# alex-petrenko/megaverse

Measured on AMD Instinct MI355X. Metric: agent observations/sec (whole node), TowerBuilding 128x128 obs, random policy, higher is better.
Workload: dtype f32

## Files before the change

### megaverse_amd/csrc/mv_raster.hip

```cpp
#include <hip/hip_runtime.h>
#include <hip/hip_ext.h>
#include <math.h>
#include <stdlib.h>

#include <algorithm>
#include <cstring>
#include <numeric>
#include <type_traits>
#include <vector>
#include <stdio.h>

#include "../../include/megaverse_hip.h"
#include "mv_frame.h"
#include "mv_math.h"
#include "mv_raster.h"
#include "mv_rearrange.h"
#include "mv_types.h"
#include "mv_union.h"

namespace mv {

namespace {

template <bool ANYZERO>
// ... 504 lines not shown
            const int py = pyBase + TILE_H * k;
            if constexpr (CHW) put_px(frame_out<true>(obs, frame, W, H, false), px, py, rgba);
            else if (px < W && py < H) out[(size_t)py * W + px] = rgba;
        }
    }
}

namespace {

#ifndef MV_GLIST_WAVES_NP2
#define MV_GLIST_WAVES_NP2 5
#endif
#ifndef MV_GLIST_WAVES_NP1
#define MV_GLIST_WAVES_NP1 6
#endif
constexpr int GLIST_WAVES_NP2 = MV_GLIST_WAVES_NP2, GLIST_WAVES_NP1 = MV_GLIST_WAVES_NP1;
#ifndef MV_FAST_PPL_DEFAULT
#define MV_FAST_PPL_DEFAULT 2
#endif
constexpr float SPEC_COS2 = 0.97f * 0.97f;

#ifndef MV_PIXEL_PLAIN
#define PIXEL_STORE(dst, v) __builtin_nontemporal_store((uint32_t)(v), &(dst))
#else
#define PIXEL_STORE(dst, v) ((dst) = (v))
#endif

struct FastArgs {
    const unsigned char *vis_hdr;
    const Prim *vis_prims;
    const short4 *vis_rects;
    const int *hist, *list;
    int num_agents, vis_stride, frames;
    const float *stage_rewards, *stage_true;
    const uint8_t *stage_done;
    float *pub_rewards, *pub_true;
    uint8_t *pub_done;
    int pub_n;
#ifdef MV_RASTER_TIMING
    unsigned long long *rdbg;
#endif
    int *hist_done;
    int wg_total;
    int tail_div, tail_split;
    int planar;
};

__device__ __forceinline__ void fast_publish(const FastArgs &fa, int blk)
{
    if (fa.pub_n == 0) return;
    const int i = blk * (int)blockDim.x + (int)threadIdx.x;
    if (i >= fa.pub_n) return;
    fa.pub_rewards[i] = fa.stage_rewards[i];
    const int e = i / fa.num_agents;
    if (fa.stage_done[e]) fa.pub_true[i] = fa.stage_true[i];
    if (i < fa.pub_n / fa.num_agents) fa.pub_done[i] = fa.stage_done[i];
}

__device__ __forceinline__ unsigned long long uniform_u64(unsigned long long v)
{
    const unsigned lo = (unsigned)__builtin_amdgcn_readfirstlane((unsigned)v), hi = (unsigned)__builtin_amdgcn_readfirstlane((unsigned)(v >> 32));
    return ((unsigned long long)hi << 32) | lo;
}

__device__ __forceinline__ float uniform_f32(float v)
{
// ... 155 lines not shown
    unsigned rgba = 0xff000000u;
    if (best <= (KEY_FAR | POS_MASK)) {
        const int pos = (int)(best & POS_MASK);
        rgba = shade_rec<SHAPES>(s_vis[2 * pos], s_vis[2 * pos + 1], __uint_as_float((best & ~POS_MASK) + KEY_NEAR),
                                 bn, s_hdr, camv, viewer, dw, inv, dcx, dcy, a2, ldc);
    }
    return rgba;
}

struct FastFrame { int frame, part, viewer, nVis, split; };

__host__ __device__ inline int tail_frames(int frames, int div) { return (frames / div) & ~7; }

template <int MAXVIS, bool GLIST = false, int NT = 256>
__device__ __forceinline__ FastFrame fast_prologue(const FastArgs &fa, int blk, int W, int H, int split,
                                                   float4 *s_vis, short4 *s_rect, float *s_hdr, float4 *s_col,
                                                   float4 *s_row, float2 *s_rowq, float *s_colq, unsigned char *s_cls = nullptr)
{
    const int A = fa.num_agents;
    const int tid = threadIdx.x, lane = tid & 63, wave = __builtin_amdgcn_readfirstlane(tid >> 6);
    int position, part;
    {
        int b = blk, first = 0, frames = fa.frames;
        if (fa.tail_div) {
            const int q = tail_frames(frames, fa.tail_div), head = frames - q;
            if (b < split * head) frames = head;
            else { b -= split * head; first = head; split = fa.tail_split; frames = q; }
        }
        const int per = 8 * split, group = b / per, r = b - group * per;
        position = group * 8 + (r & 7); part = r >> 3;
        if (group * 8 + 8 > frames) { const int nf = frames - group * 8; position = group * 8 + r % nf; part = r / nf; }
        position += first;
    }
    __shared__ int s_wsum[4], s_frame, s_lastWG;
    {
        static_assert(LPT_SUBS == 4, "the bin's counters are read as one int4");
        const bool binThread = NT == 256 || tid < LPT_BUCKETS;
        const int4 c0 = binThread ? *reinterpret_cast<const int4 *>(fa.hist + (LPT_BUCKETS - 1 - tid) * LPT_SUBS) : make_int4(0, 0, 0, 0);
        const int h = (c0.x + c0.y) + (c0.z + c0.w);
        int x = h;
#pragma unroll
        for (int off = 1; off < 64; off <<= 1) {
            const int y = __shfl_up(x, off, 64);
            if (lane >= off) x += y;
        }
        if (lane == 63 && binThread) s_wsum[wave] = x;
        __syncthreads();
        int base = 0;
        for (int w = 0; w < wave && w < 4; ++w) base += s_wsum[w];
        const int end = base + x, start = end - h;
        if (binThread && position >= start && position < end) {
            const int cs[LPT_SUBS] = {c0.x, c0.y, c0.z, c0.w};
            int off = position - start, sub = 0;
#pragma unroll
            for (int q = 0; q < LPT_SUBS - 1; ++q)
                if (sub == q && off >= cs[q]) { off -= cs[q]; sub = q + 1; }
            s_frame = fa.list[(size_t)((LPT_BUCKETS - 1 - tid) * LPT_SUBS + sub) * lpt_sub_capacity(fa.frames) + off];
        }
        __syncthreads();
    }
#ifdef MV_HIST_FENCE
    if (tid == 0) s_lastWG = fa.hist_done != nullptr && __hip_atomic_fetch_add(fa.hist_done, 1, __ATOMIC_ACQ_REL, __HIP_MEMORY_SCOPE_AGENT) == fa.wg_total - 1;
#else
    if (tid == 0) s_lastWG = fa.hist_done != nullptr && __hip_atomic_fetch_add(fa.hist_done, 1, __ATOMIC_RELAXED, __HIP_MEMORY_SCOPE_AGENT) == fa.wg_total - 1;
#endif
    const int frame = __builtin_amdgcn_readfirstlane(s_frame);
    const int viewer = frame % A;
    const float *gh = reinterpret_cast<const float *>(fa.vis_hdr + (size_t)frame * FRAME_HDR_BYTES);
    const int nVis = __builtin_amdgcn_readfirstlane(min(__float_as_int(gh[FH_COUNT]), (int)MAXVIS));

    if (tid < FH_FLOATS) s_hdr[tid] = gh[tid];
    {
        const float4 *src = reinterpret_cast<const float4 *>(fa.vis_prims + (size_t)frame * fa.vis_stride);
        if (!GLIST) for (int i = tid; i < nVis * 2; i += NT) s_vis[i] = src[i];
        else
            for (int i = tid; i < nVis; i += NT) {
                const unsigned ml = __float_as_uint(reinterpret_cast<const float *>(src)[8 * i + 3]);
                const unsigned fl = (ml >> 4) & 15u;
                s_cls[i] = (ml & 15u) != (unsigned)PRIM_BOX ? 4 : fl == 0u ? 0 : fl > (unsigned)MAX_AGENTS ? (unsigned char)(fl - (unsigned)MAX_AGENTS) : 4;
            }
        const short4 *rs = fa.vis_rects + (size_t)frame * fa.vis_stride;
        for (int i = tid; i < nVis; i += NT) s_rect[i] = rs[i];
        const float *c = gh + FH_CAM + FH_CAM_STRIDE * viewer + 3;
        for (int i = tid; i < W; i += NT) {
            const float dcx = (((float(i) + 0.5f) / float(W)) * 2.0f - 1.0f) * TAN_HALF_FOV;
            s_col[i] = make_float4(dcx, c[0] * dcx, c[3] * dcx, c[6] * dcx);
            s_colq[i] = dcx * dcx;
        }
        for (int j = tid; j < H; j += NT) {
            const float dcy = (((float(j) + 0.5f) / float(H)) * 2.0f - 1.0f) * TAN_HALF_FOV_Y;
            s_row[j] = make_float4(dcy, c[1] * dcy, c[4] * dcy, c[7] * dcy);
            s_rowq[j] = make_float2(dcy * dcy + 1.0f, 4.0f * dcy - 2.0f);
        }
// ... 17 lines not shown
    const float tf = __builtin_fminf(__builtin_fminf(fx * inv.x, fy * inv.y), fz * inv.z);
    const unsigned key = ((__float_as_uint(tn) - KEY_NEAR) & depthMask) | (unsigned)pos;
    return tn <= tf ? key : ~0u;
}

template <unsigned POS_MASK, int NP, int SGN = -1>
__device__ __forceinline__ void box_run(unsigned long long m, int k, const V3 (&inv)[NP], const float4 *s_vis, unsigned (&best)[NP])
{
    if (!m) return;
    int p0 = __ffsll((long long)m) - 1 + 64 * k, p1 = 0;
    m &= m - 1;
    float4 lo0 = s_vis[2 * p0], hi0 = s_vis[2 * p0 + 1], lo1 = lo0, hi1 = hi0;
    unsigned depthMask = ~POS_MASK;
    asm volatile("" : "+v"(depthMask));
    for (;;) {
        bool more = m != 0ull;
        if (more) { p1 = __ffsll((long long)m) - 1 + 64 * k; m &= m - 1; lo1 = s_vis[2 * p1]; hi1 = s_vis[2 * p1 + 1]; }
#pragma unroll
        for (int j = 0; j < NP; ++j) best[j] = min(best[j], SGN >= 0 ? box_key_signed<POS_MASK, (SGN >= 0 ? SGN : 0)>(inv[j], lo0, hi0, p0, depthMask)
             : box_key<POS_MASK>(inv[j], lo0, hi0, p0, depthMask));
        if (!more) break;
        more = m != 0ull;
        if (more) { p0 = __ffsll((long long)m) - 1 + 64 * k; m &= m - 1; lo0 = s_vis[2 * p0]; hi0 = s_vis[2 * p0 + 1]; }
#pragma unroll
        for (int j = 0; j < NP; ++j) best[j] = min(best[j], SGN >= 0 ? box_key_signed<POS_MASK, (SGN >= 0 ? SGN : 0)>(inv[j], lo1, hi1, p1, depthMask)
             : box_key<POS_MASK>(inv[j], lo1, hi1, p1, depthMask));
        if (!more) break;
    }
}

}

constexpr float PLANAR_MARGIN = 2e-4f;
enum : unsigned { TC_EMPTY = 0, TC_PLANAR = 1, TC_PLANAR_SPEC = 2, TC_OVERLAY = 3, TC_GENERAL = 4 };
constexpr int CLS_MAX_TILES = 128;

template <int TH, int NT>
__device__ __forceinline__ void classify_tiles(uint4 *s_tile, float4 *s_line, const float4 *s_vis, const short4 *s_rect,
                                               const float *s_hdr, const float *camv, int nVis, unsigned long long wb0,
                                               int W, int H, int part, int split, int tilesX, int numTiles,
                                                       int perWG, bool overlayOn, int *s_cnt, unsigned *s_txy, bool bulkClear)
{
    constexpr int NW = NT / 64;
    constexpr int PPR = 16 / NW;
    const int tid = threadIdx.x, lane = tid & 63, wave = __builtin_amdgcn_readfirstlane(tid >> 6);
    if (tid < CLS_MAX_TILES) s_tile[tid] = make_uint4(0u, 0u, 0u, 0u);
    if (tid < 8) s_cnt[tid] = 0;
    const float sx = 2.0f * TAN_HALF_FOV / float(W), ox = (1.0f / float(W) - 1.0f) * TAN_HALF_FOV;
    const float sy = 2.0f * TAN_HALF_FOV_Y / float(H), oy = (1.0f / float(H) - 1.0f) * TAN_HALF_FOV_Y;
    const int q = lane & 15, es = lane >> 4;
    const int ek = min(q >> 2, 2);
    int em = ek + 1 + ((q >> 1) & 1);
    em = em >= 3 ? em - 3 : em;
    const bool ehi = q & 1, eactive = q < 12;
    const float Ak = camv[3 + 3 * ek] * sx, Bk = camv[4 + 3 * ek] * sy, Ck = (camv[3 + 3 * ek] * ox + camv[4 + 3 * ek] * oy) - camv[5 + 3 * ek];
    const float Am = camv[3 + 3 * em] * sx, Bm = camv[4 + 3 * em] * sy, Cm = (camv[3 + 3 * em] * ox + camv[4 + 3 * em] * oy) - camv[5 + 3 * em];
    float4 *myLines = s_line + 16 * PPR * wave;
    constexpr float WX = float(TILE_W - 1), WY = float(TH - 1);
    __syncthreads();
    constexpr int CH = CLS_MAX_TILES / 64;
    int tX0[CH], tY0[CH], tX1[CH], tY1[CH];
    bool tvalid[CH];
    unsigned mlo[CH], mhi[CH], cover[CH];
#pragma unroll
    for (int c = 0; c < CH; ++c) {
        const int u = 64 * c + lane;
        const int tile = ((u >> 2) * split + part) * 4 + (u & 3);
        tvalid[c] = u < perWG && tile < numTiles;
        const int tyi = tile / tilesX, txi = tile - tyi * tilesX;
        tX0[c] = txi * TILE_W; tY0[c] = tyi * TH;
        tX1[c] = min(tX0[c] + TILE_W, W) - 1; tY1[c] = min(tY0[c] + TH, H) - 1;
        mlo[c] = mhi[c] = cover[c] = 0u;
    }
    for (int base = PPR * wave; base < nVis; base += 16) {
        const int P = min(base + min(es, PPR - 1), nVis - 1);
        const bool isBox = es < PPR && base + es < nVis && ((wb0 >> P) & 1ull) != 0ull;
        const float4 lo4 = s_vis[2 * P], hi4 = s_vis[2 * P + 1];
        const float lok = ek == 0 ? lo4.x : ek == 1 ? lo4.y : lo4.z, hik = ek == 0 ? hi4.x : ek == 1 ? hi4.y : hi4.z;
        const float lom = em == 0 ? lo4.x : em == 1 ? lo4.y : lo4.z, him = em == 0 ? hi4.x : em == 1 ? hi4.y : hi4.z;
        const float bnd = ehi ? him : lom;
        const bool cand = isBox && eactive && (lok > 0.0f || hik < 0.0f);
        const float pk = lok > 0.0f ? lok : hik;
        const float far1 = (__builtin_fmaxf(__builtin_fabsf(lo4.x), __builtin_fabsf(hi4.x)) + __builtin_fmaxf(__builtin_fabsf(lo4.y), __builtin_fabsf(hi4.y))) +
                           __builtin_fmaxf(__builtin_fabsf(lo4.z), __builtin_fabsf(hi4.z));
        const bool coverOK = cand && __builtin_fabsf(pk) >= 4.0f * NEAR_Z && far1 <= 0.5f * FAR_Z;
        const float sg = ((pk > 0.0f) != ehi) ? 1.0f : -1.0f;
        const float ea = sg * (pk * Am - bnd * Ak), eb = sg * (pk * Bm - bnd * Bk), ec = sg * (pk * Cm - bnd * Ck);
        const float mg = PLANAR_MARGIN * (__builtin_fabsf(pk) + __builtin_fabsf(bnd));
        const float cin = ((ec + __builtin_fminf(0.0f, ea * WX)) + __builtin_fminf(0.0f, eb * WY)) - mg;
        const float span = (__builtin_fabsf(ea) * WX + __builtin_fabsf(eb) * WY) + 2.0f * mg;
        if (es < PPR) myLines[lane] = cand ? make_float4(ea, eb, cin, span) : make_float4(0.0f, 0.0f, -1.0f, 0.0f);
        const unsigned long long candMask = __ballot(cand), coverMask = __ballot(coverOK);
        __builtin_amdgcn_fence(__ATOMIC_RELEASE, "wavefront");
        __builtin_amdgcn_wave_barrier();
        __builtin_amdgcn_fence(__ATOMIC_ACQUIRE, "wavefront");
#pragma unroll
        for (int sl = 0; sl < PPR; ++sl) {
            const int Q = base + sl;
            if (Q >= nVis) break;
            const uint2 rr = *reinterpret_cast<const uint2 *>(&s_rect[Q]);
            const bool worldBox = (wb0 >> Q) & 1ull;
#pragma unroll
            for (int c = 0; c < CH; ++c) {
                if (64 * c >= perWG) break;
                const bool ov = tvalid[c] & ((int)(rr.x & 0xffffu) <= tX1[c]) & ((int)(rr.x >> 16) >= tX0[c])
                                             & ((int)(rr.y & 0xffffu) <= tY1[c]) & ((int)(rr.y >> 16) >= tY0[c]);
                if (!__any(ov)) continue;
                bool hit = ov;
                unsigned cov = 0u;
                if (worldBox) {
                    const float fx0 = float(tX0[c]), fy0 = float(tY0[c]);
                    bool missAll = true;
#pragma unroll
                    for (int f = 0; f < 3; ++f) {
                        if (!((candMask >> (16 * sl + 4 * f)) & 1ull)) continue;
                        bool ins = true, mis = false;
#pragma unroll
                        for (int e = 0; e < 4; ++e) {
                            const float4 L = myLines[16 * sl + 4 * f + e];
                            const float g = __builtin_fmaf(L.x, fx0, __builtin_fmaf(L.y, fy0, L.z));
                            ins = ins && g >= 0.0f;
                            mis = mis || g + L.w <= 0.0f;
                        }
                        if (ins && ((coverMask >> (16 * sl + 4 * f)) & 1ull)) cov = (unsigned)f + 1u;
                        missAll = missAll && mis;
                    }
                    hit = ov && !missAll;
                }
                if (hit) {
                    if (Q < 32) mlo[c] |= 1u << Q; else mhi[c] |= 1u << (Q - 32);
                    cover[c] |= cov;
                }
            }
        }
        __builtin_amdgcn_fence(__ATOMIC_RELEASE, "wavefront");
        __builtin_amdgcn_wave_barrier();
        __builtin_amdgcn_fence(__ATOMIC_ACQUIRE, "wavefront");
    }
#pragma unroll
    for (int c = 0; c < CH; ++c)
        if (tvalid[c]) {
            const int u = 64 * c + lane;
            if (mlo[c]) atomicOr(&s_tile[u].x, mlo[c]);
            if (mhi[c]) atomicOr(&s_tile[u].y, mhi[c]);
            if (cover[c]) atomicOr(&s_tile[u].z, cover[c]);
        }
    __syncthreads();
    {
        const float hx = 0.5f * WX * sx, hy = 0.5f * WY * sy;
        const float r2 = hx * hx + hy * hy;
        const float cosT = 0.965f * __builtin_amdgcn_sqrtf(__builtin_fmaxf(1.0f - r2, 0.0f)) - 0.2623f * __builtin_amdgcn_sqrtf(r2);
        const bool usable = r2 < 0.5f && cosT > 0.0f;
        const float cosT2 = cosT * cosT;
        const float L0 = s_hdr[FH_LREL + 0], L1 = s_hdr[FH_LREL + 1], L2 = s_hdr[FH_LREL + 2];
        const unsigned long long nonBox = __ballot(lane < nVis && (__float_as_uint(s_vis[2 * min(lane, max(nVis - 1, 0))].w) & 15u) != (unsigned)PRIM_BOX);
#pragma unroll
        for (int c = 0; c < CH; ++c) {
            if (wave != (c % NW) || !tvalid[c]) continue;
            const int u = 64 * c + lane;
            const uint4 tc = s_tile[u];
            const unsigned long long m = ((unsigned long long)tc.y << 32) | tc.x, wbm = m & wb0, others = m & ~wb0;
            unsigned info = TC_GENERAL;
            if (m == 0ull) info = TC_EMPTY;
            else if (wbm != 0ull && (wbm & (wbm - 1ull)) == 0ull && tc.z != 0u) {
                const int pos = __ffsll((long long)wbm) - 1, k = (int)tc.z - 1;
                if (others == 0ull) {
                    bool maybe = true;
                    if (usable) {
                        const float lok = reinterpret_cast<const float *>(s_vis)[8 * pos + k], hik = reinterpret_cast<const float *>(s_vis)[8 * pos + 4 + k];
                        const float plane = lok > 0.0f ? lok : hik;
                        const float m0 = k == 0 ? 2.0f * plane - L0 : L0, m1 = k == 1 ? 2.0f * plane - L1 : L1, m2 = k == 2 ? 2.0f * plane - L2 : L2;
                        const float xc = float(tX0[c]) + 0.5f * WX, yc = float(tY0[c]) + 0.5f * WY;
                        const float dcx = sx * xc + ox, dcy = sy * yc + oy;
                        const float d0 = (camv[3] * dcx + camv[4] * dcy) - camv[5], d1 = (camv[6] * dcx + camv[7] * dcy) - camv[8],
// ... 5 lines not shown
                    info = (maybe ? (unsigned)TC_PLANAR_SPEC : (unsigned)TC_PLANAR) | ((unsigned)k << 3) | ((unsigned)pos << 5);
                } else if ((others & nonBox) == 0ull && overlayOn) info = (unsigned)TC_OVERLAY | ((unsigned)k << 3) | ((unsigned)pos << 5);
            }
            if (info == TC_GENERAL) {
                const float xa = float(tX0[c]), xb = float(tX1[c]), ya = float(tY0[c]), yb = float(tY1[c]);
                unsigned sg = 8u;
#pragma unroll
                for (int a = 0; a < 3; ++a) {
                    const float Aa = camv[3 + 3 * a] * sx, Ba = camv[4 + 3 * a] * sy, Ca = (camv[3 + 3 * a] * ox + camv[4 + 3 * a] * oy) - camv[5 + 3 * a];
                    const float v00 = __builtin_fmaf(Aa, xa, __builtin_fmaf(Ba, ya, Ca)), v10 = __builtin_fmaf(Aa, xb, __builtin_fmaf(Ba, ya, Ca));
                    const float v01 = __builtin_fmaf(Aa, xa, __builtin_fmaf(Ba, yb, Ca)), v11 = __builtin_fmaf(Aa, xb, __builtin_fmaf(Ba, yb, Ca));
                    const float lo4 = __builtin_fminf(__builtin_fminf(v00, v10), __builtin_fminf(v01, v11)),
                                                      hi4 = __builtin_fmaxf(__builtin_fmaxf(v00, v10), __builtin_fmaxf(v01, v11));
                    if (hi4 < -1e-4f) sg |= 1u << a;
                    else if (!(lo4 > 1e-4f)) sg = 0u;
                    if (sg == 0u) break;
                }
                info |= sg << 11;
            }
            s_tile[u].w = info;
            const unsigned tclass = info & 7u, cat = tclass == TC_GENERAL ? 0u : tclass == TC_OVERLAY ? 1u
                    : tclass == TC_PLANAR_SPEC ? 2u : tclass == TC_PLANAR ? 3u : 4u;
            const bool runs = tclass == TC_PLANAR || tclass == TC_PLANAR_SPEC || (tclass == TC_EMPTY && !bulkClear);
            const unsigned txy = (unsigned)tX0[c] | ((unsigned)tY0[c] << 16);
            const unsigned prevInfo = (unsigned)__shfl_up((int)info, 1, 64), prevTxy = (unsigned)__shfl_up((int)txy, 1, 64);
            const bool natHead = !runs || lane == 0 || prevInfo != info || prevTxy + (unsigned)TILE_W != txy;
            const unsigned long long nat = __ballot(natHead), below = nat & ((2ull << lane) - 1ull);
            const int posInRun = lane - (63 - __clzll((long long)below));
            const bool head = natHead || (posInRun & 7) == 0;
            const unsigned long long heads = __ballot(head), valid = __ballot(true), above = lane < 63 ? heads >> (lane + 1) : 0ull;
            const int nextHead = above ? lane + __ffsll((long long)above) : 64;
            const int len = min(nextHead, (int)__popcll(valid)) - lane;
            s_tile[u].z = head ? cat | ((unsigned)len << 3) | ((unsigned)atomicAdd(&s_cnt[cat], 1) << 7) : 7u;
            s_txy[u] = txy;
        }
        __syncthreads();
    }
}

template <int NP, bool SPEC, class PO>
__device__ __forceinline__ void planar_run(int pos, int k, int n, const float4 *s_vis, const float *s_hdr, const float4 *s_col, const float4 *s_row,
                                           const float2 *s_rowq, const float *s_colq, float nzk, int tx0, int ty0, int lane, const PO &po)
{
    const int W = po.W, H = po.H;
    const float lok = uniform_f32(reinterpret_cast<const float *>(s_vis)[8 * pos + k]),
                                  hik = uniform_f32(reinterpret_cast<const float *>(s_vis)[8 * pos + 4 + k]);
    const float plane = lok > 0.0f ? lok : hik;
    const unsigned color = (unsigned)__builtin_amdgcn_readfirstlane(__float_as_uint(reinterpret_cast<const float *>(s_vis)[8 * pos + 7]));
    const float cr = float((color >> 16) & 255u), cg = float((color >> 8) & 255u), cb = float(color & 255u);
    const float lk = uniform_f32(s_hdr[FH_LREL + k]);
    const float lks = plane > 0.0f ? lk : 0.0f - lk;
    int lpx = lane;
    asm volatile("" : "+v"(lpx));
    const int lx = lpx & (TILE_W - 1), py0 = ty0 + lpx / TILE_W;
    float rowk[NP];
    float2 rq[NP];
#pragma unroll
    for (int j = 0; j < NP; ++j) {
        const int pyc = min(py0 + TILE_H * j, H - 1);
        rowk[j] = reinterpret_cast<const float *>(s_row)[4 * pyc + 1 + k];
        rq[j] = s_rowq[pyc];
    }
#pragma unroll 1
    for (int q = 0; q < n; ++q) {
        const int px = tx0 + TILE_W * q + lx, pxc = min(px, W - 1);
        const float colk = reinterpret_cast<const float *>(s_col)[4 * pxc + 1 + k];
        const float cq = s_colq[pxc];
// ... 148 lines not shown
    const unsigned long long wbm = mv0 & wb0;
    switch (signs) {
    case 8: box_run<POS_MASK, NP, 0>(wbm, 0, inv, s_vis, best); break;
    case 9: box_run<POS_MASK, NP, 1>(wbm, 0, inv, s_vis, best); break;
    case 10: box_run<POS_MASK, NP, 2>(wbm, 0, inv, s_vis, best); break;
    case 11: box_run<POS_MASK, NP, 3>(wbm, 0, inv, s_vis, best); break;
    case 12: box_run<POS_MASK, NP, 4>(wbm, 0, inv, s_vis, best); break;
    case 13: box_run<POS_MASK, NP, 5>(wbm, 0, inv, s_vis, best); break;
    case 14: box_run<POS_MASK, NP, 6>(wbm, 0, inv, s_vis, best); break;
    case 15: box_run<POS_MASK, NP, 7>(wbm, 0, inv, s_vis, best); break;
    default: box_run<POS_MASK, NP>(wbm, 0, inv, s_vis, best); break;
    }
    unsigned long long rest = mv0 & ~wb0;
    while (rest) {
        const int pos = __ffsll((long long)rest) - 1;
        rest &= rest - 1;
#pragma unroll
        for (int j = 0; j < NP; ++j) {
            V3 n = v3(0, 0, 0);
            const unsigned key = fast_other<SHAPES, POS_MASK>(pos, s_vis, s_hdr, camv, viewer, dw[j], dcx, dcy[j], n);
            if (key < best[j]) { best[j] = key; bn[j] = n; }
        }
    }
#pragma unroll
    for (int j = 0; j < NP; ++j) {
        const unsigned rgba = fast_shade<SHAPES, POS_MASK>(best[j], bn[j], s_vis, s_hdr, camv, viewer, dw[j], inv[j], dcx, dcy[j], a2[j], ldc[j]);
        put_px(po, px, py0 + TILE_H * j, rgba);
    }
}

constexpr int fast_lds_bytes(int maxvis) { return 40 * maxvis + 4 * FH_FLOATS; }
constexpr int glist_lds_bytes(int maxvis) { return 9 * maxvis + 4 * FH_FLOATS; }

#ifdef MV_RASTER_TIMING
#define RT_COUNT(i, n) do { const unsigned long long n_ = (unsigned long long)(n); if (fa.rdbg && lane == 0) atomicAdd(fa.rdbg + (size_t)16384 * 4 * 8 + (i), n_); } while (0)
#else
#define RT_COUNT(i, n) do { } while (0)
#endif
template <bool SHAPES, unsigned POS_MASK, int NP, bool LISTED, class PO>
__device__ __forceinline__ void classified_tile(const FastArgs &fa, const int u, const int tx0, const int ty0, const uint4 *s_tile,
                                                const float4 *s_vis, const float *s_hdr, const float *camv, int viewer,
                                            const float4 *s_col, const float4 *s_row, const float2 *s_rowq,
                                                    const float *s_colq, float nzm0, float nzm1, float nzm2, unsigned long long wb0,
                                            int lane, const PO &po)
{
    const unsigned info = (unsigned)__builtin_amdgcn_readfirstlane(s_tile[u].w), tclass = info & 7u;
    const int run = LISTED ? (int)(((unsigned)__builtin_amdgcn_readfirstlane(s_tile[u].z) >> 3) & 15u) : 1;
    RT_COUNT(0, run);
    if (tclass == TC_EMPTY) {
        RT_COUNT(1, run);
        for (int q = 0; q < run; ++q) clear_tile<NP>(po, tx0 + TILE_W * q, ty0, lane);
        return;
    }
    if (LISTED && tclass <= TC_PLANAR_SPEC) {
        const int k = (int)((info >> 3) & 3u), posA = (int)(info >> 5);
        const float nzk = k == 0 ? nzm0 : k == 1 ? nzm1 : nzm2;
        RT_COUNT(2, run);
        RT_COUNT(12, tclass == TC_PLANAR ? run : 0);
        if (tclass == TC_PLANAR) planar_run<NP, false>(posA, k, run, s_vis, s_hdr, s_col, s_row, s_rowq, s_colq, nzk, tx0, ty0, lane, po);
        else planar_run<NP, true>(posA, k, run, s_vis, s_hdr, s_col, s_row, s_rowq, s_colq, nzk, tx0, ty0, lane, po);
        return;
    }
    int lpx = lane;
    asm volatile("" : "+v"(lpx));
    const int px = tx0 + (lpx & (TILE_W - 1)), py0 = ty0 + lpx / TILE_W;
    if (tclass <= TC_OVERLAY) {
#if defined(MV_RASTER_DEBUG_SKIP) && MV_RASTER_DEBUG_SKIP == 3
        return;
#endif
        const int k = (int)((info >> 3) & 3u), posA = (int)(info >> 5);
        const float nzk = k == 0 ? nzm0 : k == 1 ? nzm1 : nzm2;
// ... 43 lines not shown
    unsigned long long rt_[6];
    rt_[0] = __builtin_amdgcn_s_memtime(); rt_[5] = __builtin_amdgcn_s_memrealtime();
#define RT_MARK(i) rt_[i] = __builtin_amdgcn_s_memtime()
#else
#define RT_MARK(i) do { } while (0)
#endif
    fast_publish(fa, blk);
    const FastFrame ff = fast_prologue<MAXVIS, false, NT>(fa, blk, W, H, split, s_vis, s_rect, s_hdr, s_col, s_row, s_rowq, s_colq);
    RT_MARK(1);
    const int frame = ff.frame, part = ff.part, viewer = ff.viewer, nVis = ff.nVis;
    split = ff.split;

    const float *camv = s_hdr + FH_CAM + FH_CAM_STRIDE * viewer;
    const float nzm0 = uniform_f32(-camv[3 + 2]), nzm1 = uniform_f32(-camv[3 + 5]), nzm2 = uniform_f32(-camv[3 + 8]);
    uint32_t *out = obs + (size_t)frame * W * H;
    const int tilesX = (W + TILE_W - 1) / TILE_W, tilesY = (H + TH - 1) / TH;
    const int numTiles = tilesX * tilesY;
    PixOutT<CHW> po;
    if constexpr (CHW) po = frame_out<true>(obs, frame, W, H, (W % TILE_W) == 0 && (H % TH) == 0);
    else {
        po.rsrc = __builtin_amdgcn_make_buffer_rsrc(out,  0, W * H * 4, 0x00020000);
        po.W = W; po.H = H; po.W4 = 4 * W;
        po.edgeless = (W % TILE_W) == 0 && (H % TH) == 0;
    }

    uint2 rr0 = make_uint2(0u, 0u);
    if (NP == 1) rr0 = *reinterpret_cast<const uint2 *>(&s_rect[min(lane, max(nVis - 1, 0))]);
    const unsigned long long wb0 = uniform_u64(*reinterpret_cast<const unsigned long long *>(s_hdr + FH_WB));

    constexpr bool PLANAR = !HEXF && CLS;
    static_assert(!PLANAR || (MAXVIS == 256 && CLS_MAX_TILES == 128), "classification tables: 256 edge functions + 128 tiles = 192 records");
    float4 *s_line = s_vis + 2 * 64;
    uint4 *s_tile = reinterpret_cast<uint4 *>(s_vis + 2 * 64 + 256);
    const int perWG = (numTiles - part * 4 + 4 * split - 1) / (4 * split) * 4;
    const bool cls = PLANAR && fa.planar && nVis <= 64 && perWG <= CLS_MAX_TILES && perWG >= 32;
    __shared__ int s_next;
    __shared__ int s_cnt[8];
    __shared__ unsigned s_txy[CLS_MAX_TILES];
    __shared__ unsigned short s_order[CLS_MAX_TILES], s_empty[CLS_MAX_TILES];
    if (tid == 0) s_next = NT / 64;
    int nList = 0;
#ifndef MV_TILE_LIST
#define MV_TILE_LIST 1
#endif
    constexpr bool LISTED = PLANAR && MV_TILE_LIST != 0;
    const bool bulk = LISTED && po.edgeless && (W & 3) == 0;
    if (PLANAR && cls && !LISTED) classify_tiles<TH, NT>(s_tile, s_line, s_vis, s_rect, s_hdr, camv, nVis, wb0, W, H,
        part, split, tilesX, numTiles, perWG, fa.planar != 2, s_cnt, s_txy, true);
    else if (PLANAR && cls) {
        classify_tiles<TH, NT>(s_tile, s_line, s_vis, s_rect, s_hdr, camv, nVis, wb0, W, H, part, split,
                               tilesX, numTiles, perWG, fa.planar != 2, s_cnt, s_txy, bulk);
        const int c0 = s_cnt[0], c1 = s_cnt[1], c2 = s_cnt[2], c3 = s_cnt[3], nE = s_cnt[4];
        nList = __builtin_amdgcn_readfirstlane(c0 + c1 + c2 + c3 + (bulk ? 0 : nE));
        if (tid < CLS_MAX_TILES) {
            const int tile = ((tid >> 2) * split + part) * 4 + (tid & 3);
            if (tid < perWG && tile < numTiles) {
                const unsigned z = s_tile[tid].z, cat = z & 7u, place = z >> 7;
                const int base = cat == 0u ? 0 : cat == 1u ? c0 : cat == 2u ? c0 + c1 : cat == 3u ? c0 + c1 + c2 : c0 + c1 + c2 + c3;
                if (cat == 4u && bulk) s_empty[place] = (unsigned short)tid;
                else if (cat != 7u) s_order[base + (int)place] = (unsigned short)tid;
            }
        }
        __syncthreads();
        if (bulk) {
            constexpr int CPT = TH * 4;
            static_assert(NT % CPT == 0, "threads per empty tile");
            const int sub = tid % CPT;
            unsigned c = 0xff000000u;
            asm volatile("" : "+v"(c));
            const v4u_t v = {c, c, c, c};
            if constexpr (CHW) {
                const v4u_t z = {0u, 0u, 0u, 0u};
                const int c = sub / TH;
                const unsigned inoff = (unsigned)__mul24(c, po.plane) + (unsigned)__mul24(sub - c * TH, po.W);
                if (c < 3)
                    for (int e = tid / CPT; e < nE; e += NT / CPT) {
                        const unsigned txy = s_txy[s_empty[e]];
                        __builtin_amdgcn_raw_buffer_store_b128(z, po.rsrc, (unsigned)__mul24((int)(txy >> 16), po.W) + (txy & 0xffffu) + inoff, 0, PLANAR_AUX);
                    }
            } else {
            const unsigned inoff = (unsigned)__mul24(sub >> 2, po.W4) + (unsigned)(sub & 3) * 16u;
            for (int e = tid / CPT; e < nE; e += NT / CPT) {
                const unsigned txy = s_txy[s_empty[e]];
                __builtin_amdgcn_raw_buffer_store_b128(v, po.rsrc, (unsigned)__mul24((int)(txy >> 16), po.W4) + (txy & 0xffffu) * 4u + inoff, 0, PIXEL_AUX);
// ... 539 lines not shown
    f.hist_done = a.done_base[s] ? a.done_base[s] + par : nullptr;
    f.pub_rewards = a.pub_rewards[t][s];
    f.pub_done = a.pub_done[t][s];
    return f;
}

template <int WAVES, int NPS, bool CHW = false>
__global__ __launch_bounds__(256, WAVES) void raster_union_batch_kernel(UnionBatchArgs a, int W, int H)
{
    int j = 0, r = (int)blockIdx.x;
    while (r >= a.per_tick) { r -= a.per_tick; ++j; }
    int s = 0;
#pragma unroll
    for (int i = 1; i < MAX_UNION; ++i)
        if (i < a.n && r >= a.first[i]) s = i;
    const int blk = r - a.first[s];
    if (j == 0)
        for (int t = 0; t < a.k; ++t) fast_publish(union_batch_args(a, s, t), blk);
    constexpr int LDS = fast_lds_bytes(VIS_SMALL) > glist_lds_bytes(VIS_XL) ? fast_lds_bytes(VIS_SMALL) : glist_lds_bytes(VIS_XL);
    __shared__ __attribute__((aligned(16))) unsigned char s_buf[LDS];
    FastArgs fa = union_batch_args(a, s, j);
    fa.pub_n = 0;
    if (a.large[s]) raster_glist_body<VIS_XL, true, true, 1, CHW>(fa, a.obs[j][s], W, H, a.split_large, blk, s_buf);
    else raster_fast_body<VIS_SMALL, true, false, NPS, MV_UNION_CLS, 256, CHW>(fa, a.obs[j][s], W, H, a.split_small, blk, s_buf);
}

#ifdef MV_RASTER_TIMING
static unsigned long long *g_rdbg = nullptr;
static void rdbg_dump()
{
    if (!g_rdbg) return;
    (void)hipDeviceSynchronize();
    {
        unsigned long long c[16];
        const bool got = hipMemcpy(c, g_rdbg + (size_t)16384 * 4 * 8, sizeof(c), hipMemcpyDeviceToHost) == hipSuccess;
        if (got && c[10])
            fprintf(stderr, "long-list census (all launches): tiles %llu, rounds of 64 list positions walked %.2f of %.2f per tile, early stops (every pixel "
                    "nearer than the next class) in %.3f of the tiles, "
                            "%.1f primitives met per tile; tiles that met nothing %.3f, one world-frame box only %.3f, two primitives %.3f, 3-5: %.3f, 6 and "
                                    "more: %.3f\n",
                    c[10], double(c[11]) / c[10], double(c[12]) / c[10], double(c[15]) / c[10], double(c[13]) / c[10],
                                  double(c[14]) / c[10], double(c[9]) / c[10], double(c[8]) / c[10],
                    double(c[7]) / c[10], double(c[6]) / c[10]);
        if (got && c[10])
            fprintf(stderr, "long-list census, tests: %.2f slab tests and %.2f other primitives per tile (%.2f / %.2f per tile that meets anything), %.1f of a tile's "
                    "pixels hit something\n", double(c[4]) / c[10], double(c[5]) / c[10], double(c[4]) / double(c[10] - c[14]), double(c[5]) / double(c[10] - c[14]),
                    double(c[3]) / c[10]);
        if (got && c[4] && !c[10])
            fprintf(stderr, "raster census (all launches): classified tiles %llu (empty %llu, planar %llu of which %llu without the highlight test, covered "
                    "+ overlay %llu), unclassified %llu, general-path tiles %llu: "
                            "slab tests %.2f and other primitives %.2f per tile\n",
                    c[0], c[1], c[2], c[12], c[13], c[3], c[4], double(c[5]) / c[4], double(c[6]) / c[4]);
    }
    std::vector<unsigned long long> h((size_t)16384 * 4 * 8);
    if (hipMemcpy(h.data(), g_rdbg, h.size() * 8, hipMemcpyDeviceToHost) != hipSuccess) return;
    double sumP = 0, sumC = 0, sumT = 0; size_t n = 0;
    unsigned long long r0 = ~0ull, r1 = 0;
    std::vector<double> life, endAt;
    for (size_t w = 0; w < (size_t)16384 * 4; ++w) {
        const unsigned long long *o = &h[w * 8];
        if (!o[0]) continue;
        sumP += double(o[1] - o[0]); sumC += double(o[2] - o[1]); sumT += double(o[3] - o[2]); ++n;
        r0 = std::min(r0, o[4]); r1 = std::max(r1, o[5]);
    }
    if (!n) return;
    for (size_t w = 0; w < (size_t)16384 * 4; ++w) {
        const unsigned long long *o = &h[w * 8];
        if (!o[0]) continue;
        life.push_back(double(o[5] - o[4]) * 0.01); endAt.push_back(double(o[5] - r0) * 0.01);
    }
    std::vector<double> spread;
    for (size_t g = 0; g < 16384; ++g) {
        unsigned long long lo = ~0ull, hi = 0; int k = 0;
        for (int w = 0; w < 4; ++w) { const unsigned long long *o = &h[(g * 4 + w) * 8]; if (o[0]) { lo = std::min(lo, o[5]); hi = std::max(hi, o[5]); ++k; } }
        if (k == 4) spread.push_back(double(hi - lo) * 0.01);
    }
    std::sort(spread.begin(), spread.end());
    if (!spread.empty()) fprintf(stderr, "raster timing: within a workgroup, last wave's end - first wave's end (us): mean %.1f p50 %.1f p90 %.1f max %.1f\n",
                                 std::accumulate(spread.begin(), spread.end(), 0.0) / spread.size(),
                                                 spread[spread.size() / 2], spread[spread.size() * 9 / 10], spread.back());
    {
        std::vector<std::pair<double, size_t>> byLife;
        for (size_t w = 0; w < (size_t)16384 * 4; ++w) { const unsigned long long *o = &h[w * 8]; if (o[0]) byLife.push_back({double(o[5] - o[4]) * 0.01, w}); }
        std::sort(byLife.begin(), byLife.end(), [](auto &a, auto &b) { return a.first > b.first; });
        for (size_t q = 0; q < std::min<size_t>(byLife.size(), 12); q += 1) {
// ... 25 lines not shown
            fprintf(stderr, " | start us");
            for (int d = 0; d < 10; ++d) fprintf(stderr, " %.1f", cnt[d] ? ps[d] / cnt[d] : 0.0);
            fprintf(stderr, " | nVis");
            for (int d = 0; d < 10; ++d) fprintf(stderr, " %.0f", cnt[d] ? pn[d] / cnt[d] : 0.0);
            fprintf(stderr, "\n");
        }
    }
    std::sort(life.begin(), life.end()); std::sort(endAt.begin(), endAt.end());
    auto pct = [](const std::vector<double> &v, double p) { return v[std::min(v.size() - 1, (size_t)(p * v.size()))]; };
    fprintf(stderr, "raster timing (last launch, %zu waves): cycles per wave: prologue %.0f, classification %.0f, tile loop %.0f | wave life us: mean %.1f "
            "p10 %.1f p50 %.1f p90 %.1f max %.1f | "
                    "launch %.1f us; waves ended by (us): 10%% %.1f, 25%% %.1f, 50%% %.1f, 75%% %.1f, 90%% %.1f, 99%% %.1f\n",
            n, sumP / n, sumC / n, sumT / n, std::accumulate(life.begin(), life.end(), 0.0) / life.size(),
                                                             pct(life, 0.1), pct(life, 0.5), pct(life, 0.9), life.back(),
            double(r1 - r0) * 0.01, pct(endAt, 0.1), pct(endAt, 0.25), pct(endAt, 0.5), pct(endAt, 0.75), pct(endAt, 0.9), pct(endAt, 0.99));
}
#endif

static void self_clear(struct FastArgs &fa, const GymView &gv, int workgroups);

static FastArgs fast_args_of(const GymView &gv, const PublishTo *publish)
{
    const int frames = gv.num_envs * gv.num_agents;
    FastArgs fa;
    fa.vis_hdr = gv.vis_hdr; fa.vis_prims = reinterpret_cast<const Prim *>(gv.vis_prims); fa.vis_rects = reinterpret_cast<const short4 *>(gv.vis_rects);
    fa.hist = gv.lpt_hist + gv.lpt_parity * (LPT_BUCKETS * LPT_SUBS); fa.list = gv.lpt_list; fa.num_agents = gv.num_agents;
                                             fa.vis_stride = gv.vis_stride; fa.frames = frames;
    fa.stage_rewards = gv.rewards; fa.stage_true = gv.true_objective; fa.stage_done = gv.done;
    fa.pub_rewards = publish ? publish->rewards : nullptr; fa.pub_true = publish ? publish->true_objective
            : nullptr; fa.pub_done = publish ? publish->done : nullptr;
    fa.pub_n = publish ? frames : 0;
    const char *pe = getenv("MV_PLANAR");
    fa.planar = pe && *pe ? atoi(pe) : 1;
    fa.tail_div = 0; fa.tail_split = 0;
    fa.hist_done = nullptr; fa.wg_total = 0;
#ifdef MV_RASTER_TIMING
    if (!g_rdbg && hipMalloc((void **)&g_rdbg, (size_t)(16384 * 4 * 8 + 64) * 8) == hipSuccess) { (void)hipMemset(g_rdbg,
        0, (size_t)(16384 * 4 * 8 + 64) * 8); atexit(rdbg_dump); }
    fa.rdbg = g_rdbg;
#endif
    return fa;
}

static void self_clear(FastArgs &fa, const GymView &gv, int workgroups)
{
    if (!gv.lpt_no_clear) return;
    fa.hist_done = gv.lpt_hist + (size_t)gv.lpt_hists * (LPT_BUCKETS * LPT_SUBS) + gv.lpt_parity;
    fa.wg_total = workgroups;
}

static int fast_pixels_per_lane(int W, int H, bool longList = false, bool batch = false)
{
    const char *e = getenv("MV_FAST_PPL");
    if (e && *e) return atoi(e) >= 2 ? 2 : 1;
    return (!longList || batch) && MV_FAST_PPL_DEFAULT >= 2 && W * H >= 8192 ? 2 : 1;
}

static int fast_split(int W, int H, int np, int frames, bool longList = false, bool batch = false)
{
    const int ftiles = ((W + TILE_W - 1) / TILE_W) * ((H + TILE_H * np - 1) / (TILE_H * np));
    const int want = ((np >= 2 ? 2048 : 4096) + frames - 1) / std::max(frames, 1), lo = (batch || frames >= 4096) && np >= 2
                      && !longList ? 1 : batch && !longList ? 1 : np >= 2 ? 2 : 4, hi = np >= 2 ? 8 : 16;
    int split = lo;
    while (split < hi && split < want) split <<= 1;
    while (split > 1 && ftiles < 4 * split * (longList ? 1 : 2)) split >>= 1;
    return split;
// ... 230 lines not shown
```

Before: 29.27 million.

## Compact box-tile pairs into per-wave rings for lane-dense tile classification

Tile classification now collects overlapping (world box, tile) pairs into a per-wave LDS ring and tests edge functions for 64 pairs at a time, instead of each lane testing its own tiles against every box with many lanes idle. This targets divergence and idle lanes in the classify loop. It adds ring bookkeeping, extra wave barriers and shared-memory atomics, and it is on by default through the MV_CLS_PAIRS environment variable. Separately, the LPT frame lookup now scans the 256 histogram bins with a single wave, four bins per lane, which removes one workgroup barrier and the cross-wave sum.

```diff
diff --git a/megaverse_amd/csrc/mv_raster.hip b/megaverse_amd/csrc/mv_raster.hip
--- a/megaverse_amd/csrc/mv_raster.hip
+++ b/megaverse_amd/csrc/mv_raster.hip
@@ -560,6 +560,7 @@
     const short4 *vis_rects;
     const int *hist, *list;
     int num_agents, vis_stride, frames;
+    int cls_pairs;
     const float *stage_rewards, *stage_true;
     const uint8_t *stage_done;
     float *pub_rewards, *pub_true;
@@ -781,33 +782,40 @@
         if (group * 8 + 8 > frames) { const int nf = frames - group * 8; position = group * 8 + r % nf; part = r / nf; }
         position += first;
     }
-    __shared__ int s_wsum[4], s_frame, s_lastWG;
-    {
+    __shared__ int s_frame, s_lastWG;
+    if (wave == 0) {
         static_assert(LPT_SUBS == 4, "the bin's counters are read as one int4");
-        const bool binThread = NT == 256 || tid < LPT_BUCKETS;
-        const int4 c0 = binThread ? *reinterpret_cast<const int4 *>(fa.hist + (LPT_BUCKETS - 1 - tid) * LPT_SUBS) : make_int4(0, 0, 0, 0);
-        const int h = (c0.x + c0.y) + (c0.z + c0.w);
+        static_assert(LPT_BUCKETS == 4 * 64, "one wave: four cost bins per lane");
+        const int4 *hp = reinterpret_cast<const int4 *>(fa.hist + (LPT_BUCKETS - 1 - 4 * lane) * LPT_SUBS);
+        const int4 ca = hp[0], cb = hp[-1], cc = hp[-2], cd = hp[-3];
+        const int ha = (ca.x + ca.y) + (ca.z + ca.w), hb = (cb.x + cb.y) + (cb.z + cb.w), hc = (cc.x + cc.y) + (cc.z + cc.w), hd = (cd.x + cd.y) + (cd.z + cd.w);
+        const int h = (ha + hb) + (hc + hd);
         int x = h;
 #pragma unroll
         for (int off = 1; off < 64; off <<= 1) {
             const int y = __shfl_up(x, off, 64);
             if (lane >= off) x += y;
         }
-        if (lane == 63 && binThread) s_wsum[wave] = x;
-        __syncthreads();
-        int base = 0;
-        for (int w = 0; w < wave && w < 4; ++w) base += s_wsum[w];
-        const int end = base + x, start = end - h;
-        if (binThread && position >= start && position < end) {
+        const int start = x - h;
+        if (position >= start && position < x) {
+            int off = position - start, bq = 0;
+            int4 c0 = ca;
+            if (off >= ha) {
+                off -= ha; bq = 1; c0 = cb;
+                if (off >= hb) {
+                    off -= hb; bq = 2; c0 = cc;
+                    if (off >= hc) { off -= hc; bq = 3; c0 = cd; }
+                }
+            }
             const int cs[LPT_SUBS] = {c0.x, c0.y, c0.z, c0.w};
-            int off = position - start, sub = 0;
+            int sub = 0;
 #pragma unroll
             for (int q = 0; q < LPT_SUBS - 1; ++q)
                 if (sub == q && off >= cs[q]) { off -= cs[q]; sub = q + 1; }
-            s_frame = fa.list[(size_t)((LPT_BUCKETS - 1 - tid) * LPT_SUBS + sub) * lpt_sub_capacity(fa.frames) + off];
-        }
-        __syncthreads();
-    }
+            s_frame = fa.list[(size_t)((LPT_BUCKETS - 1 - (4 * lane + bq)) * LPT_SUBS + sub) * lpt_sub_capacity(fa.frames) + off];
+        }
+    }
+    __syncthreads();
 #ifdef MV_HIST_FENCE
     if (tid == 0) s_lastWG = fa.hist_done != nullptr && __hip_atomic_fetch_add(fa.hist_done, 1, __ATOMIC_ACQ_REL, __HIP_MEMORY_SCOPE_AGENT) == fa.wg_total - 1;
 #else
@@ -891,17 +899,61 @@
 }
 
 constexpr float PLANAR_MARGIN = 2e-4f;
+#ifdef MV_RASTER_TIMING
+#define RT_COUNT(i, n) do { const unsigned long long n_ = (unsigned long long)(n); if (fa.rdbg && lane == 0) atomicAdd(fa.rdbg + (size_t)16384 * 4 * 8 + (i), n_); } while (0)
+#else
+#define RT_COUNT(i, n) do { } while (0)
+#endif
 enum : unsigned { TC_EMPTY = 0, TC_PLANAR = 1, TC_PLANAR_SPEC = 2, TC_OVERLAY = 3, TC_GENERAL = 4 };
 constexpr int CLS_MAX_TILES = 128;
 
+template <int PPR, class pair_t>
+__device__ __forceinline__ void cls_pair_pass(const pair_t *ring, int head, int n, int cap, const float4 *myLines, const unsigned *s_txy, uint4 *s_tile,
+                                              unsigned long long candMask, unsigned long long coverMask, int base, int lane)
+{
+    __builtin_amdgcn_fence(__ATOMIC_RELEASE, "wavefront");
+    __builtin_amdgcn_wave_barrier();
+    __builtin_amdgcn_fence(__ATOMIC_ACQUIRE, "wavefront");
+    if (lane < n) {
+        const unsigned e = ring[(head + lane) & (cap - 1)];
+        const unsigned u = e & 127u, sl = (e >> 7) & (unsigned)(PPR - 1);
+        const unsigned txy = s_txy[u];
+        const float fx0 = float(txy & 0xffffu), fy0 = float(txy >> 16);
+        const unsigned cm = (unsigned)(candMask >> (16u * sl)), cvm = (unsigned)(coverMask >> (16u * sl));
+        const float4 *L4 = myLines + 16u * sl;
+        bool missAll = true;
+        unsigned cov = 0u;
+#pragma unroll
+        for (int f = 0; f < 3; ++f) {
+            if (!__any((cm >> (4 * f)) & 1u)) continue;
+            bool ins = true, mis = false;
+#pragma unroll
+            for (int q = 0; q < 4; ++q) {
+                const float4 L = L4[4 * f + q];
+                const float g = __builtin_fmaf(L.x, fx0, __builtin_fmaf(L.y, fy0, L.z));
+                ins = ins && g >= 0.0f;
+                mis = mis || g + L.w <= 0.0f;
+            }
+            if (ins && ((cvm >> (4 * f)) & 1u)) cov = (unsigned)f + 1u;
+            missAll = missAll && mis;
+        }
+        if (!missAll) {
+            const unsigned Q = (unsigned)base + sl;
+            atomicOr(&s_tile[u].x + (Q >> 5), 1u << (Q & 31u));
+            if (cov) atomicOr(&s_tile[u].z, cov);
+        }
+    }
+}
+
 template <int TH, int NT>
-__device__ __forceinline__ void classify_tiles(uint4 *s_tile, float4 *s_line, const float4 *s_vis, const short4 *s_rect,
-                                               const float *s_hdr, const float *camv, int nVis, unsigned long long wb0,
+__device__ __forceinline__ void classify_tiles(const FastArgs &fa, uint4 *s_tile, float4 *s_line, unsigned char *s_pair, const float4 *s_vis,
+                                               const short4 *s_rect, const float *s_hdr, const float *camv, int nVis, unsigned long long wb0,
                                                int W, int H, int part, int split, int tilesX, int numTiles,
-                                                       int perWG, bool overlayOn, int *s_cnt, unsigned *s_txy, bool bulkClear)
+                                               int perWG, int *s_cnt, unsigned *s_txy, bool bulkClear)
 {
     constexpr int NW = NT / 64;
     constexpr int PPR = 16 / NW;
+    const bool overlayOn = fa.planar != 2;
     const int tid = threadIdx.x, lane = tid & 63, wave = __builtin_amdgcn_readfirstlane(tid >> 6);
     if (tid < CLS_MAX_TILES) s_tile[tid] = make_uint4(0u, 0u, 0u, 0u);
     if (tid < 8) s_cnt[tid] = 0;
@@ -916,11 +968,9 @@
     const float Am = camv[3 + 3 * em] * sx, Bm = camv[4 + 3 * em] * sy, Cm = (camv[3 + 3 * em] * ox + camv[4 + 3 * em] * oy) - camv[5 + 3 * em];
     float4 *myLines = s_line + 16 * PPR * wave;
     constexpr float WX = float(TILE_W - 1), WY = float(TH - 1);
-    __syncthreads();
     constexpr int CH = CLS_MAX_TILES / 64;
     int tX0[CH], tY0[CH], tX1[CH], tY1[CH];
     bool tvalid[CH];
-    unsigned mlo[CH], mhi[CH], cover[CH];
 #pragma unroll
     for (int c = 0; c < CH; ++c) {
         const int u = 64 * c + lane;
@@ -929,8 +979,20 @@
         const int tyi = tile / tilesX, txi = tile - tyi * tilesX;
         tX0[c] = txi * TILE_W; tY0[c] = tyi * TH;
         tX1[c] = min(tX0[c] + TILE_W, W) - 1; tY1[c] = min(tY0[c] + TH, H) - 1;
-        mlo[c] = mhi[c] = cover[c] = 0u;
-    }
+        if (wave == (c % NW) && tvalid[c]) s_txy[u] = (unsigned)tX0[c] | ((unsigned)tY0[c] << 16);
+    }
+    __syncthreads();
+    constexpr int PAIR_CAP = 128;
+    typedef typename std::conditional<(PPR > 2), unsigned short, unsigned char>::type pair_t;
+    static_assert(PPR <= 2 || (PPR <= 4 && sizeof(pair_t) == 2), "a pair entry: local tile (7 bits) | slot << 7");
+    static_assert(CLS_MAX_TILES <= 128 && NW * PAIR_CAP * sizeof(pair_t) <= (256 - 64) * sizeof(short4), "the rings live behind a classified frame's 64 rectangles");
+    pair_t *myPairs = reinterpret_cast<pair_t *>(s_pair) + PAIR_CAP * wave;
+    const bool pairs = fa.cls_pairs != 0;
+    if (pairs && wave == 0) RT_COUNT(18, 1);
+    int pHead = 0, pTail = 0;
+    unsigned mlo[CH], mhi[CH], cover[CH];
+#pragma unroll
+    for (int c = 0; c < CH; ++c) mlo[c] = mhi[c] = cover[c] = 0u;
     for (int base = PPR * wave; base < nVis; base += 16) {
         const int P = min(base + min(es, PPR - 1), nVis - 1);
         const bool isBox = es < PPR && base + es < nVis && ((wb0 >> P) & 1ull) != 0ull;
@@ -953,6 +1015,43 @@
         __builtin_amdgcn_fence(__ATOMIC_RELEASE, "wavefront");
         __builtin_amdgcn_wave_barrier();
         __builtin_amdgcn_fence(__ATOMIC_ACQUIRE, "wavefront");
+        if (pairs) {
+#pragma unroll
+            for (int sl = 0; sl < PPR; ++sl) {
+                const int Q = base + sl;
+                if (Q >= nVis) break;
+                const uint2 rr = *reinterpret_cast<const uint2 *>(&s_rect[Q]);
+                const bool worldBox = (wb0 >> Q) & 1ull;
+                if (worldBox && !((candMask >> (16 * sl)) & 0x111ull)) continue;
+#pragma unroll
+                for (int c = 0; c < CH; ++c) {
+                    if (64 * c >= perWG) break;
+                    const bool ov = tvalid[c] & ((int)(rr.x & 0xffffu) <= tX1[c]) & ((int)(rr.x >> 16) >= tX0[c])
+                                                 & ((int)(rr.y & 0xffffu) <= tY1[c]) & ((int)(rr.y >> 16) >= tY0[c]);
+                    const unsigned long long om = __ballot(ov);
+                    if (!om) continue;
+                    if (!worldBox) {
+                        if (ov) atomicOr(&s_tile[64 * c + lane].x + (Q >> 5), 1u << (Q & 31));
+                        continue;
+                    }
+                    const int at = (int)__builtin_amdgcn_mbcnt_hi((unsigned)(om >> 32), __builtin_amdgcn_mbcnt_lo((unsigned)om, (unsigned)pTail));
+                    if (ov) myPairs[at & (PAIR_CAP - 1)] = (pair_t)((64 * c + lane) | (sl << 7));
+                    pTail += (int)__popcll(om);
+                    RT_COUNT(16, __popcll(om));
+                    if (pTail - pHead >= 64) {
+                        cls_pair_pass<PPR>(myPairs, pHead, 64, PAIR_CAP, myLines, s_txy, s_tile, candMask, coverMask, base, lane);
+                        pHead += 64;
+                        RT_COUNT(17, 1);
+                    }
+                }
+            }
+            while (pHead < pTail) {
+                const int n = min(64, pTail - pHead);
+                cls_pair_pass<PPR>(myPairs, pHead, n, PAIR_CAP, myLines, s_txy, s_tile, candMask, coverMask, base, lane);
+                pHead += n;
+                RT_COUNT(17, 1);
+            }
+        } else {
 #pragma unroll
         for (int sl = 0; sl < PPR; ++sl) {
             const int Q = base + sl;
@@ -992,13 +1091,14 @@
                 }
             }
         }
+        }
         __builtin_amdgcn_fence(__ATOMIC_RELEASE, "wavefront");
         __builtin_amdgcn_wave_barrier();
         __builtin_amdgcn_fence(__ATOMIC_ACQUIRE, "wavefront");
     }
 #pragma unroll
     for (int c = 0; c < CH; ++c)
-        if (tvalid[c]) {
+        if (!pairs && tvalid[c]) {
             const int u = 64 * c + lane;
             if (mlo[c]) atomicOr(&s_tile[u].x, mlo[c]);
             if (mhi[c]) atomicOr(&s_tile[u].y, mhi[c]);
@@ -1070,7 +1170,6 @@
             const int nextHead = above ? lane + __ffsll((long long)above) : 64;
             const int len = min(nextHead, (int)__popcll(valid)) - lane;
             s_tile[u].z = head ? cat | ((unsigned)len << 3) | ((unsigned)atomicAdd(&s_cnt[cat], 1) << 7) : 7u;
-            s_txy[u] = txy;
         }
         __syncthreads();
     }
@@ -1285,11 +1384,6 @@
 constexpr int fast_lds_bytes(int maxvis) { return 40 * maxvis + 4 * FH_FLOATS; }
 constexpr int glist_lds_bytes(int maxvis) { return 9 * maxvis + 4 * FH_FLOATS; }
 
-#ifdef MV_RASTER_TIMING
-#define RT_COUNT(i, n) do { const unsigned long long n_ = (unsigned long long)(n); if (fa.rdbg && lane == 0) atomicAdd(fa.rdbg + (size_t)16384 * 4 * 8 + (i), n_); } while (0)
-#else
-#define RT_COUNT(i, n) do { } while (0)
-#endif
 template <bool SHAPES, unsigned POS_MASK, int NP, bool LISTED, class PO>
 __device__ __forceinline__ void classified_tile(const FastArgs &fa, const int u, const int tx0, const int ty0, const uint4 *s_tile,
                                                 const float4 *s_vis, const float *s_hdr, const float *camv, int viewer,
@@ -1399,6 +1493,7 @@
     static_assert(!PLANAR || (MAXVIS == 256 && CLS_MAX_TILES == 128), "classification tables: 256 edge functions + 128 tiles = 192 records");
     float4 *s_line = s_vis + 2 * 64;
     uint4 *s_tile = reinterpret_cast<uint4 *>(s_vis + 2 * 64 + 256);
+    unsigned char *s_pair = reinterpret_cast<unsigned char *>(s_rect + 64);
     const int perWG = (numTiles - part * 4 + 4 * split - 1) / (4 * split) * 4;
     const bool cls = PLANAR && fa.planar && nVis <= 64 && perWG <= CLS_MAX_TILES && perWG >= 32;
     __shared__ int s_next;
@@ -1412,11 +1507,11 @@
 #endif
     constexpr bool LISTED = PLANAR && MV_TILE_LIST != 0;
     const bool bulk = LISTED && po.edgeless && (W & 3) == 0;
-    if (PLANAR && cls && !LISTED) classify_tiles<TH, NT>(s_tile, s_line, s_vis, s_rect, s_hdr, camv, nVis, wb0, W, H,
-        part, split, tilesX, numTiles, perWG, fa.planar != 2, s_cnt, s_txy, true);
+    if (PLANAR && cls && !LISTED) classify_tiles<TH, NT>(fa, s_tile, s_line, s_pair, s_vis, s_rect, s_hdr, camv, nVis, wb0, W, H,
+        part, split, tilesX, numTiles, perWG, s_cnt, s_txy, true);
     else if (PLANAR && cls) {
-        classify_tiles<TH, NT>(s_tile, s_line, s_vis, s_rect, s_hdr, camv, nVis, wb0, W, H, part, split,
-                               tilesX, numTiles, perWG, fa.planar != 2, s_cnt, s_txy, bulk);
+        classify_tiles<TH, NT>(fa, s_tile, s_line, s_pair, s_vis, s_rect, s_hdr, camv, nVis, wb0, W, H, part, split,
+                               tilesX, numTiles, perWG, s_cnt, s_txy, bulk);
         const int c0 = s_cnt[0], c1 = s_cnt[1], c2 = s_cnt[2], c3 = s_cnt[3], nE = s_cnt[4];
         nList = __builtin_amdgcn_readfirstlane(c0 + c1 + c2 + c3 + (bulk ? 0 : nE));
         if (tid < CLS_MAX_TILES) {
@@ -2022,7 +2117,7 @@
     if (!g_rdbg) return;
     (void)hipDeviceSynchronize();
     {
-        unsigned long long c[16];
+        unsigned long long c[19];
         const bool got = hipMemcpy(c, g_rdbg + (size_t)16384 * 4 * 8, sizeof(c), hipMemcpyDeviceToHost) == hipSuccess;
         if (got && c[10])
             fprintf(stderr, "long-list census (all launches): tiles %llu, rounds of 64 list positions walked %.2f of %.2f per tile, early stops (every pixel "
@@ -2041,6 +2136,10 @@
                     "+ overlay %llu), unclassified %llu, general-path tiles %llu: "
                             "slab tests %.2f and other primitives %.2f per tile\n",
                     c[0], c[1], c[2], c[12], c[13], c[3], c[4], double(c[5]) / c[4], double(c[6]) / c[4]);
+        if (got && c[18] && !c[10])
+            fprintf(stderr, "pair census (all launches): classifying workgroups %llu, (box, tile) pairs enumerated %llu = %.1f per workgroup, pair passes "
+                    "%llu = %.2f per workgroup, %.1f pairs per pass of 64 lanes\n",
+                    c[18], c[16], double(c[16]) / c[18], c[17], double(c[17]) / c[18], c[17] ? double(c[16]) / c[17] : 0.0);
     }
     std::vector<unsigned long long> h((size_t)16384 * 4 * 8);
     if (hipMemcpy(h.data(), g_rdbg, h.size() * 8, hipMemcpyDeviceToHost) != hipSuccess) return;
@@ -2132,6 +2231,8 @@
     fa.pub_n = publish ? frames : 0;
     const char *pe = getenv("MV_PLANAR");
     fa.planar = pe && *pe ? atoi(pe) : 1;
+    const char *cp = getenv("MV_CLS_PAIRS");
+    fa.cls_pairs = cp && *cp ? atoi(cp) != 0 : 1;
     fa.tail_div = 0; fa.tail_split = 0;
     fa.hist_done = nullptr; fa.wg_total = 0;
 #ifdef MV_RASTER_TIMING
```

New measurement: 29.56 million (median of 6 runs). About the same (+1.0%).
